# yz-cnsdqz/PSI-release

Measured on AMD Instinct MI355X. Metric: fitting iters/sec (SMPL-X+SDF+Chamfer), PROX-E batch=32, higher is better.
Workload: dtype f32

## Files before the change

psi-release_amd/csrc/fit.hip:

```cpp
#include "psi_internal.h"
#ifdef PSI_HEAD_STOPS
__device__ int psi_dbg_sstop;
#define PSI_SSTOP(k) do { if (psi_dbg_sstop == (k)) return; } while (0)
__device__ int psi_dbg_pstop;
#define PSI_PSTOP(k) do { if (psi_dbg_pstop == (k)) asm volatile("s_endpgm"); } while (0)
#define PSI_TRACE(lo, hi) PsiBlockTrace trace_((lo), (hi))
__device__ unsigned long long psi_dbg_tl[4 * 8192];
struct PsiBlockTrace {
    unsigned long long t0;
    int kind;
    int sel_lo, sel_hi;
    __device__ PsiBlockTrace(int lo = 9, int hi = 10) : t0(wall_clock64()), kind(0), sel_lo(lo), sel_hi(hi) {}
    __device__ ~PsiBlockTrace()
    {
        const unsigned bid = blockIdx.y * gridDim.x + blockIdx.x;
        if (psi_dbg_sstop < sel_lo || psi_dbg_sstop > sel_hi || threadIdx.x != 0 || bid >= 8192) return;
        unsigned long long *o = psi_dbg_tl + 4 * (size_t)bid;
        o[0] = t0;
        o[1] = wall_clock64();
        o[2] = (unsigned long long)__builtin_amdgcn_s_getreg((31 << 11) | 4) | ((unsigned long long)__builtin_amdgcn_s_getreg((31 << 11) | 20) << 32);
        o[3] = (unsigned long long)kind;
    }
};
extern "C" int psi_dbg_timeline(unsigned long long *out, int nblocks)
// ... 43 lines not shown
    const int *vid;
    const int *cs_ptr, *cs_idx;
    const int *cs_first;
    const float *scene, *sdf, *gmin, *gmax;
    const float *sdf_brick;
    const float *Wct;
    float *x, *xhr, *cam, *adam_m, *adam_v;
    int *step;
    float *h1, *h2, *o6, *betas20, *pose, *transl, *verts, *og, *gq, *fpart, *penpart, *recpart, *vppart;
    float *cverts;
    float *g_betas, *g_pose, *g_transl, *g_rot;
    unsigned long long *hx_o6, *hx_gh1;
    unsigned *hx_epoch;
    int *hx_err;
    int hc;
#ifdef PSI_HEAD_STOPS
    int stop_h, stop_t;
#define HSTOP(k) do { if (f.stop_h == (k)) return; } while (0)
#define TSTOP(k) do { if (f.stop_t == (k)) return; } while (0)
#else
#define HSTOP(k)
#define TSTOP(k)
#endif
    int *nn_hint;
    float *history;
    int max_hist;
    int fused_bwd, ncp, ncp3;
    float *glc, *gvpc, *vpc;
    float *gtc_part;
#ifndef PSI_GV_SLOTS
#define PSI_GV_SLOTS 1024
#endif
    unsigned *gvbits;
    const float *dirs_ch;
    const float *WTt_c;
    float *gA_part, *gfeat_part;
    float *spb;
    int nsv, nsv_c, nsn_m, nsn_c, spm, spc;
};

__device__ __forceinline__ float leaky(float v, float slope) { return v > 0.0f ? v : v * slope; }

__device__ __forceinline__ void gs_forward(const float *x6, float *R)
{
    float a1[3] = {x6[0], x6[2], x6[4]}, a2[3] = {x6[1], x6[3], x6[5]};
    float n1 = fmaxf(sqrtf(a1[0] * a1[0] + a1[1] * a1[1] + a1[2] * a1[2]), 1e-12f);
    float b1[3] = {a1[0] / n1, a1[1] / n1, a1[2] / n1};
    float d = b1[0] * a2[0] + b1[1] * a2[1] + b1[2] * a2[2];
    float u[3] = {a2[0] - d * b1[0], a2[1] - d * b1[1], a2[2] - d * b1[2]};
    float n2 = fmaxf(sqrtf(u[0] * u[0] + u[1] * u[1] + u[2] * u[2]), 1e-12f);
    float b2[3] = {u[0] / n2, u[1] / n2, u[2] / n2};
    float b3[3] = {b1[1] * b2[2] - b1[2] * b2[1], b1[2] * b2[0] - b1[0] * b2[2], b1[0] * b2[1] - b1[1] * b2[0]};
    for (int r = 0; r < 3; r++) {
        R[r * 3 + 0] = b1[r];
        R[r * 3 + 1] = b2[r];
        R[r * 3 + 2] = b3[r];
    }
}

__device__ __forceinline__ void gs_backward(const float *x6, const float *gR, float *g6)
{
    float a1[3] = {x6[0], x6[2], x6[4]}, a2[3] = {x6[1], x6[3], x6[5]};
    float n1 = fmaxf(sqrtf(a1[0] * a1[0] + a1[1] * a1[1] + a1[2] * a1[2]), 1e-12f);
    float b1[3] = {a1[0] / n1, a1[1] / n1, a1[2] / n1};
    float d = b1[0] * a2[0] + b1[1] * a2[1] + b1[2] * a2[2];
    float u[3] = {a2[0] - d * b1[0], a2[1] - d * b1[1], a2[2] - d * b1[2]};
// ... 327 lines not shown
#pragma unroll
            for (int a = 0; a < 3; a++) g[a] = neg[n] ? g[a] : 0.0f;
            s[n] = neg[n] ? -val : 0.0f;
        }
        if (gl) {
#pragma unroll
            for (int a = 0; a < 3; a++) gm[n][a] = g[a];
            return;
        }
        psi_st(og + (size_t)b * Vpad * 4, (unsigned)v * 16u, f4{g[0], g[1], g[2], 0.0f});
    }
    __device__ __forceinline__ void backward(int n, int b, unsigned v12, const psi_f2 (&T2)[6], const float *C)
    {
        if (!gl) return;
        const float gx = gm[n][0], gy = gm[n][1], gz = gm[n][2];
        float lx = gx, ly = gy, lz = gz;
        if (C) {
            lx = psi_dot3(C[0], C[4], C[8], gx, gy, gz);
            ly = psi_dot3(C[1], C[5], C[9], gx, gy, gz);
            lz = psi_dot3(C[2], C[6], C[10], gx, gy, gz);
        }
        psi_st(gl + (size_t)b * Npad, v12, psi_p3{lx, ly, lz});
        const float vx = psi_dot3(T2[0].x, T2[2].x, T2[4].x, lx, ly, lz), vy = psi_dot3(T2[0].y, T2[2].y, T2[4].y, lx, ly, lz),
                    vz = psi_dot3(T2[1].x, T2[3].x, T2[5].x, lx, ly, lz);
        psi_st(gvp + (size_t)b * Npad, v12, psi_p3{vx, vy, vz});
        gvmax = fmaxf(gvmax, fmaxf(fabsf(vx), fmaxf(fabsf(vy), fabsf(vz))));
        gs[n][0] = lx; gs[n][1] = ly; gs[n][2] = lz;
    }
    __device__ __forceinline__ void finish(int n, int b, int vblock, int nvb)
    {
        __shared__ psi_f2 red[PSI_SKIN_BLK / 64];
        __shared__ float red3[PSI_SKIN_BLK / 64][3];
        __shared__ float redm[PSI_SKIN_BLK / 64];
        const float ws = psi_wave_sum(s[n]);
        const float wc = (float)(int)__builtin_popcountll(__builtin_amdgcn_ballot_w64(neg[n]));
        if ((threadIdx.x & 63) == 0) red[threadIdx.x >> 6] = (psi_f2){ws, wc};
        if (gl) {
            const float sx = psi_wave_sum(gs[n][0]), sy = psi_wave_sum(gs[n][1]), sz = psi_wave_sum(gs[n][2]);
            float mx = gvmax;
#pragma unroll
            for (int o2 = 32; o2 > 0; o2 >>= 1) mx = fmaxf(mx, __shfl_xor(mx, o2, 64));
            if ((threadIdx.x & 63) == 0) {
                red3[threadIdx.x >> 6][0] = sx;
                red3[threadIdx.x >> 6][1] = sy;
                red3[threadIdx.x >> 6][2] = sz;
                redm[threadIdx.x >> 6] = mx;
            }
        }
        __syncthreads();
        if (gl && threadIdx.x == 64) {
            float mx = redm[0];
#pragma unroll
            for (int w = 1; w < PSI_SKIN_BLK / 64; w++) mx = fmaxf(mx, redm[w]);
#ifndef PSI_NO_GVMAX_ATOMIC
            if (mx > 0.0f) atomicMax(gmaxp + (blockIdx.x & (PSI_GV_SLOTS - 1)), __float_as_uint(mx));
#endif
        }
        if (threadIdx.x == 0) {
            psi_f2 a = red[0];
#pragma unroll
            for (int w = 1; w < PSI_SKIN_BLK / 64; w++) a += red[w];
            *(psi_f2 *)(penpart + ((size_t)b * nvb + vblock) * 2) = a;
        }
        if (gl && threadIdx.x < 3) {
            float a = 0.0f;
#pragma unroll
            for (int w = 0; w < PSI_SKIN_BLK / 64; w++) a += red3[w][threadIdx.x];
            gtp[((size_t)vblock * B + b) * 4 + threadIdx.x] = a;
        }
    }
};

static inline SdfPenEpilogue make_sdf_epilogue(const FitDev &f, const PsiSdfGrid &G, bool contact_vertices_only = false, const PsiLbsView *bwd = nullptr)
{
    SdfPenEpilogue e = {G, f.sdf, f.gmin, f.gmax, f.og, f.penpart, f.D, f.align_corners, f.Vpad, contact_vertices_only ? f.cs_first : nullptr,
                        {0.0f, 0.0f}, {false, false}, f.cverts, f.cs_ptr, f.cs_idx, f.n_c, nullptr, nullptr, nullptr, 0, f.B, {}, {}, 0.0f, f.gvbits};
    if (bwd) {
        e.gl = bwd->gl;
        e.gvp = bwd->g_vp;
        e.gtp = bwd->gt_part_w;
        e.Npad = bwd->m.Npad;
    }
    return e;
}

struct ContactSkinSrc {
    FitDev f;
    LbsDev m;
    const float *As, *v_posed;
    psi_f2 (*sA)[6];
    psi_f2 st[2];
    float ct;
    int v;
    float px, py, pz;
    float *sCT;
    static constexpr int NWQ = PSI_JP / 4 - 2, NWE = 10;
    f4 wq[NWE];
    int jslot;
    float (*sTR)[9] = nullptr;
    float gvm = 0.0f;
    float gs[3] = {0.0f, 0.0f, 0.0f};
// ... 94 lines not shown
            wsum3[threadIdx.x >> 6][1] = sy;
            wsum3[threadIdx.x >> 6][2] = sz;
            wmax[threadIdx.x >> 6] = mx;
        }
        __syncthreads();
        if (threadIdx.x == 64) {
            float m2 = wmax[0];
#pragma unroll
            for (int w = 1; w < psikd::QBLK / 64; w++) m2 = fmaxf(m2, wmax[w]);
#ifndef PSI_NO_GVMAX_ATOMIC
            if (m2 > 0.0f) atomicMax(f.gvbits + PSI_GV_SLOTS + (blockIdx.x & (PSI_GV_SLOTS - 1)), __float_as_uint(m2));
#endif
        }
        if (threadIdx.x < 3) {
            float a = 0.0f;
#pragma unroll
            for (int w = 0; w < psikd::QBLK / 64; w++) a += wsum3[w][threadIdx.x];
            f.gtc_part[((size_t)b * nbx + bx) * 4 + threadIdx.x] = a;
        }
    }
};

#ifdef PSI_HEAD_STOPS
extern "C" int psi_dbg_kd_mark(unsigned long long *out, int nblocks)
{
    return (int)hipMemcpyFromSymbol(out, HIP_SYMBOL(psi_kd_mark), sizeof(unsigned long long) * 4 * (size_t)(nblocks < 8192 ? nblocks : 8192));
}
extern "C" int psi_dbg_kd_reason(int *out) { return (int)hipMemcpyFromSymbol(out, HIP_SYMBOL(psi_kd_reason), sizeof(int) * 8); }
extern "C" int psi_dbg_kd_stat(int *out, int nblocks)
{
    return (int)hipMemcpyFromSymbol(out, HIP_SYMBOL(psi_kd_stat), sizeof(int) * 4 * (size_t)(nblocks < 8192 ? nblocks : 8192));
}
#endif
template <int NB>
__global__ __launch_bounds__(256, 6) void fwd_scene_kernel(FitDev f, LbsDev m, const float *__restrict__ As, const float *__restrict__ v_posed,
                                                           psikd::KdDev T, int n_kd, int nqb, int rows, float gscale, int skin_first, SdfPenEpilogue epi)
{
    extern __shared__ int smem_i[];
#ifdef PSI_HEAD_STOPS
    if (psi_dbg_sstop == 1 && (int)blockIdx.x >= n_kd) return;
    if (psi_dbg_sstop == 2 && (int)blockIdx.x < n_kd) return;
    if (psi_dbg_sstop == 3) return;
    PsiBlockTrace trace;
    if (threadIdx.x < 4 && blockIdx.x < 8192) psi_kd_stat[4 * blockIdx.x + threadIdx.x] = 0;
    trace.kind = skin_first ? ((int)blockIdx.x >= (int)gridDim.x - n_kd) : ((int)blockIdx.x < n_kd);
#endif
    int bid = blockIdx.x;
    bool is_kd;
    if (skin_first) {
        const int n_sk = (int)gridDim.x - n_kd;
        is_kd = bid >= n_sk;
        if (is_kd) bid -= n_sk;
    } else {
        is_kd = bid < n_kd;
        if (!is_kd) bid -= n_kd;
    }
    if (is_kd) {
        const int b = bid / nqb, bx = bid % nqb;
        psikd::kd_query_body<true, false>(T, ContactSkinSrc{f, m, As, v_posed, nullptr, {}, 0.0f, 0, 0.0f, 0.0f, 0.0f, nullptr, {}, 0}, f.n_c, (float *)nullptr, (int *)nullptr, f.cconst, gscale,
                                          f.fused_bwd ? (float *)nullptr : f.gq, f.fpart, f.nn_hint, rows, (const psikd::KdDev *)nullptr, (const int *)nullptr, bx, b, nqb, smem_i);
    } else {
        const int i = bid;
        psi_skin_fwd_body<NB, PsiBlendCompact>(m, As, v_posed, f.transl, f.cam, f.B, f.verts, epi, i % f.nsdfblk, (i / f.nsdfblk) * NB, f.nsdfblk);
    }
}

__global__ void contact_weight_table_kernel(const float *__restrict__ WT, int Vpad, const int *__restrict__ vid, int n_c, int J, float *__restrict__ Wct)
{
    const int i = blockIdx.x * 256 + threadIdx.x;
    if (i >= n_c * PSI_JP) return;
    const int slot = i / PSI_JP, j = i % PSI_JP;
    Wct[i] = j < J ? WT[(size_t)j * Vpad + vid[slot]] : 0.0f;
}

__global__ __launch_bounds__(1024) void loss_finalize_kernel(FitDev f, float *stats)
{
    __shared__ float red[16];
    const int t = threadIdx.x, nt = 1024;
    auto total = [&](const float *p, int n, int stride) {
        float a0 = 0, a1 = 0, a2 = 0, a3 = 0;
        int i = t;
        for (; i + 3 * nt < n; i += 4 * nt) {
            a0 += p[(size_t)i * stride];
            a1 += p[(size_t)(i + nt) * stride];
            a2 += p[(size_t)(i + 2 * nt) * stride];
            a3 += p[(size_t)(i + 3 * nt) * stride];
        }
        for (; i < n; i += nt) a0 += p[(size_t)i * stride];
        return block_sum((a0 + a1) + (a2 + a3), red);
    };
    float s_rec = total(f.recpart, f.B, 1);
    float s_vp = total(f.vppart, f.B, 1);
    float s_f = total(f.fpart, f.B * f.nfp, 1);
    float s_pen = total(f.penpart, f.B * f.nsdfblk, 2);
    float n_pen = total(f.penpart + 1, f.B * f.nsdfblk, 2);
    if (t == 0) {
// ... 563 lines not shown
    const int bz = (int)(br % nbr), by = (int)((br / nbr) % nbr), bx = (int)(br / ((size_t)nbr * nbr));
    const int ix = min(4 * bx + (l >> 4) + (c >> 2), D - 1), iy = min(4 * by + ((l >> 2) & 3) + ((c >> 1) & 1), D - 1),
              iz = min(4 * bz + (l & 3) + (c & 1), D - 1);
    dst[i] = src[((size_t)ix * D + iy) * D + iz];
}

__global__ void adam_reset_kernel(float *m, float *v, int *step, int n)
{
    int i = blockIdx.x * 256 + threadIdx.x;
    if (i < n) { m[i] = 0.0f; v[i] = 0.0f; }
    if (i == 0) *step = 0;
}

}

#ifndef PSI_GRAPH_UNROLL
#define PSI_GRAPH_UNROLL 10
#endif
constexpr int GRAPH_UNROLL = PSI_GRAPH_UNROLL;

struct psi_fit_engine {
    FitDev d;
    PsiSdfGrid grid;
    const psi_lbs_model *lbs;
    psi_nn_index *nn_index;
    float *lbs_ws;
    PsiLbsView lv;
    void *nn_ws;
    char *blob;
    float *stats_local;
    bool merged_scene;
    bool self_skin;
    bool keep_verts;
    bool scene_skin_first;
    bool fused_bwd;
    int skin_nb;
    hipGraph_t graph, graphN, graph2N;
    hipGraphExec_t graph_exec, graphN_exec, graph2N_exec;
    bool graph_ready, graphN_ready, graph2N_ready;
    hipGraph_t g_half[2];
    hipGraphExec_t ge_half[2];
    bool half_ready[2];
    const float *half_stats[2];
    hipGraph_t g_dp[2];
    hipGraphExec_t ge_dp[2];
    bool dp_ready[2];
    const void *dp_comm;
    const float *dp_stats;
    bool dp_warm;
    bool dp_no_graph;
};

static void launch_head_fwd(const FitDev &f, const PsiLbsView &lv, hipStream_t st)
{
    const dim3 g(f.B * f.hc), blk(HB);
    switch (f.hc) {
    case 8: hipLaunchKernelGGL(head_fwd_kernel<8>, g, blk, 0, st, f, lv); break;
    case 4: hipLaunchKernelGGL(head_fwd_kernel<4>, g, blk, 0, st, f, lv); break;
    case 2: hipLaunchKernelGGL(head_fwd_kernel<2>, g, blk, 0, st, f, lv); break;
    default: hipLaunchKernelGGL(head_fwd_kernel<1>, g, blk, 0, st, f, lv); break;
    }
}

template <bool ADAM>
static void launch_head_bwd(const FitDev &f, const PsiLbsView &lv, float *g_out, hipStream_t st)
{
    const dim3 g(f.B * f.hc), blk(HB);
    switch (f.hc) {
    case 8: hipLaunchKernelGGL((head_bwd_adam_kernel<8, ADAM>), g, blk, 0, st, f, lv, g_out); break;
    case 4: hipLaunchKernelGGL((head_bwd_adam_kernel<4, ADAM>), g, blk, 0, st, f, lv, g_out); break;
    case 2: hipLaunchKernelGGL((head_bwd_adam_kernel<2, ADAM>), g, blk, 0, st, f, lv, g_out); break;
    default: hipLaunchKernelGGL((head_bwd_adam_kernel<1, ADAM>), g, blk, 0, st, f, lv, g_out); break;
    }
}

static inline bool fit_use_local_stats(const FitDev &f, bool local) { return local && f.B < PSI_SKIN_MB_MIN_B; }

static int fit_forward(psi_fit_engine *e, float *stats, hipStream_t st, bool local = false, bool finalize = true)
{
    FitDev &f = e->d;
    local = e->fused_bwd ? (local || !finalize) : fit_use_local_stats(f, local);
    launch_head_fwd(f, e->lv, st);
    PSI_CHECK_LAUNCH("head_fwd_kernel");
    psi_mark("head_fwd_kernel", st);
    int rc = psi_lbs_blend_forward(e->lbs, f.B, e->lbs_ws, st);
    if (rc) return rc;
    float gscale = f.w_contact / ((f.indep ? 1.0f : (float)f.B * (float)f.world) * (float)f.n_c);
    if (e->nn_index && e->merged_scene) {
        const psikd::KdDev T = psi_nn_index_dev(e->nn_index);
        const int nqb = f.nfp, n_kd = nqb * f.B;
        FitDev fk = f;
        if (!e->keep_verts) fk.verts = nullptr;
        if (e->skin_nb == 2)
            hipLaunchKernelGGL(fwd_scene_kernel<2>, dim3(n_kd + f.nsdfblk * psi_cdiv(f.B, 2)), dim3(256), psikd::kd_lds_bytes(T.rows), st, fk, e->lv.m,
                               e->lv.A, e->lv.v_posed, T, n_kd, nqb, T.rows, gscale, e->scene_skin_first ? 1 : 0, make_sdf_epilogue(f, e->grid, false, e->fused_bwd ? &e->lv : nullptr));
        else
            hipLaunchKernelGGL(fwd_scene_kernel<1>, dim3(n_kd + f.nsdfblk * f.B), dim3(256), psikd::kd_lds_bytes(T.rows), st, fk, e->lv.m, e->lv.A,
                               e->lv.v_posed, T, n_kd, nqb, T.rows, gscale, e->scene_skin_first ? 1 : 0, make_sdf_epilogue(f, e->grid, false, e->fused_bwd ? &e->lv : nullptr));
        PSI_CHECK_LAUNCH("fwd_scene_kernel");
        psi_mark("fwd_scene_kernel", st);
        if (local) return 0;
        hipLaunchKernelGGL(loss_finalize_kernel, dim3(1), dim3(1024), 0, st, f, stats);
        PSI_CHECK_LAUNCH("loss_finalize_kernel");
        psi_mark("loss_finalize_kernel", st);
        return 0;
    }
    const bool all_verts = !e->nn_index || (getenv("PSI_KEEP_VERTS") && getenv("PSI_KEEP_VERTS")[0] == '1');
    if (e->skin_nb == 2)
        hipLaunchKernelGGL((psi_skin_fwd_kernel<SdfPenEpilogue, 2>), dim3(f.nsdfblk, psi_cdiv(f.B, 2)), dim3(PSI_SKIN_BLK), 0, st, e->lv.m, e->lv.A,
                           e->lv.v_posed, f.transl, f.cam, f.B, f.verts, make_sdf_epilogue(f, e->grid, !all_verts));
    else
        hipLaunchKernelGGL((psi_skin_fwd_kernel<SdfPenEpilogue, 1>), dim3(f.nsdfblk, f.B), dim3(PSI_SKIN_BLK), 0, st, e->lv.m, e->lv.A,
                           e->lv.v_posed, f.transl, f.cam, f.B, f.verts, make_sdf_epilogue(f, e->grid, !all_verts));
    PSI_CHECK_LAUNCH("skin_fwd_sdf_kernel");
    psi_mark("skin_fwd_sdf_kernel", st);
    if (e->nn_index && !all_verts)
        rc = psi_nn_index_contact(e->nn_index, f.cverts, (long)f.n_c * 3, nullptr, f.B, f.n_c, f.cconst, gscale, f.gq, f.fpart, f.nn_hint, st);
    else if (e->nn_index)
        rc = psi_nn_index_contact(e->nn_index, f.verts, (long)f.V * 3, f.vid, f.B, f.n_c, f.cconst, gscale, f.gq, f.fpart, f.nn_hint, st);
    else
        rc = psi_nn_contact(f.verts, (long)f.V * 3, f.vid, f.scene, f.B, f.n_c, f.m, e->nn_ws, f.cconst, gscale, f.gq, f.fpart, nullptr, st);
    if (rc) return rc;
    if (local) return 0;
    hipLaunchKernelGGL(loss_finalize_kernel, dim3(1), dim3(1024), 0, st, f, stats);
    PSI_CHECK_LAUNCH("loss_finalize_kernel");
    psi_mark("loss_finalize_kernel", st);
    return 0;
}

static int fit_launch_stats(psi_fit_engine *e, float *stats, hipStream_t st)
{
// ... 139 lines not shown
    memcpy(b3p.data(), h_b3, NJ6 * 4);
    for (int o = 0; o < NH; o++) for (int k = 0; k < NZ; k++) W1T[(size_t)k * NH + o] = h_w1[(size_t)o * NZ + k];
    for (int o = 0; o < NH; o++) for (int k = 0; k < NH; k++) W2T[(size_t)k * NH + o] = h_w2[(size_t)o * NH + k];
    for (int o = 0; o < NJ6; o++) for (int k = 0; k < NH; k++) W3T[(size_t)k * 128 + o] = h_w3[(size_t)o * NH + k];
    std::vector<int> cs_ptr(V + 1, 0), cs_idx(f.n_c), cs_first(V, 0);
    for (int i = 0; i < f.n_c; i++) cs_ptr[h_contact_ids[i] + 1]++;
    for (int v = 0; v < V; v++) cs_ptr[v + 1] += cs_ptr[v];
    {
        std::vector<int> fill(cs_ptr.begin(), cs_ptr.end() - 1);
        for (int i = 0; i < f.n_c; i++) cs_idx[fill[h_contact_ids[i]]++] = i;
        for (int v = 0; v < V; v++)
            if (cs_ptr[v + 1] > cs_ptr[v]) cs_first[v] = cs_idx[cs_ptr[v]] | (std::min(cs_ptr[v + 1] - cs_ptr[v], 127) << 24);
    }
    struct Item { const void *src; size_t bytes; size_t off; };
    std::vector<Item> items;
    size_t o = 0;
    auto take = [&](size_t bytes) { size_t r = o; o += (bytes + 255) & ~(size_t)255; return r; };
    auto cst = [&](const void *src, size_t bytes) { size_t r = take(bytes); items.push_back({src, bytes, r}); return r; };
    size_t o_w1t = cst(W1T.data(), W1T.size() * 4), o_b1 = cst(h_b1, NH * 4), o_w2t = cst(W2T.data(), W2T.size() * 4), o_b2 = cst(h_b2, NH * 4),
           o_w3t = cst(W3T.data(), W3T.size() * 4), o_b3 = cst(b3p.data(), 128 * 4), o_w1 = cst(h_w1, (size_t)NH * NZ * 4),
           o_w2 = cst(h_w2, (size_t)NH * NH * 4), o_w3 = cst(h_w3, (size_t)NJ6 * NH * 4), o_lh = cst(h_lh_comp, (size_t)f.ncomp * 45 * 4),
           o_rh = cst(h_rh_comp, (size_t)f.ncomp * 45 * 4), o_pm = cst(h_pose_mean, (size_t)J * 3 * 4), o_vid = cst(h_contact_ids, (size_t)f.n_c * 4),
           o_cp = cst(cs_ptr.data(), cs_ptr.size() * 4), o_ci = cst(cs_idx.data(), cs_idx.size() * 4), o_cf = cst(cs_first.data(), cs_first.size() * 4), o_gmin = cst(h_gmin, 12), o_gmax = cst(h_gmax, 12);
    size_t zero_begin = o;
    size_t o_x = take((size_t)B * XD * 4), o_xhr = take((size_t)B * XD * 4), o_cam = take((size_t)B * 16 * 4), o_am = take((size_t)B * XD * 4),
           o_av = take((size_t)B * XD * 4), o_step = take(256), o_h1 = take((size_t)B * NH * 4), o_h2 = take((size_t)B * NH * 4),
           o_o6 = take((size_t)B * 128 * 4), o_b20 = take((size_t)B * NB * 4), o_pose = take((size_t)B * J * 3 * 4), o_tr = take((size_t)B * 3 * 4),
           o_verts = take((size_t)B * V * 3 * 4), o_cv = take((size_t)B * f.n_c * 3 * 4), o_og = take((size_t)B * psi_cdiv(V, 256) * 256 * 4 * 4),
           o_gq = take((size_t)B * f.n_c * 3 * 4), o_fp = take((size_t)B * f.nfp * 4), o_pp = take((size_t)B * f.nsdfblk * 2 * 4),
           o_rp = take((size_t)B * 4), o_vp = take((size_t)B * 4), o_gb = take((size_t)B * NB * 4), o_gp = take((size_t)B * J * 3 * 4),
           o_gt = take((size_t)B * 3 * 4), o_gr = take((size_t)B * J * 9 * 4), o_hist = take((size_t)f.max_hist * 4 * 4), o_stats = take(256), o_hint = take((size_t)B * f.n_c * 4);
    size_t o_hxo = take((size_t)B * f.hc * 128 * 8), o_hxg = take((size_t)B * f.hc * NH * 8), o_hxc = take((size_t)2 * B * 4);
    size_t o_wct = take((size_t)f.n_c * PSI_JP * 4);
    e->fused_bwd = e->merged_scene && !(getenv("PSI_FIT_FUSED_BWD") && getenv("PSI_FIT_FUSED_BWD")[0] == '0');
    f.fused_bwd = e->fused_bwd ? 1 : 0;
    f.ncp = psi_cdiv(f.n_c, 256) * 256;
    f.ncp3 = 3 * f.ncp;
    size_t o_glc = 0, o_gvpc = 0, o_vpc = 0, o_gtc = 0, o_gvb = 0, o_wttc = 0, o_dirsc = 0, o_gap = 0, o_gfp = 0, o_spb = 0;
    {
        PsiLbsView lv0;
        if (int rcv = psi_lbs_view(lbs, B, reinterpret_cast<float *>((uintptr_t)4096), &lv0)) { delete e; return rcv; }
        const int Kpad = lv0.m.Kpad, Npad = lv0.m.Npad, nsn = lv0.nsn;
        const int SM = Npad / 16, SC = f.ncp3 / 16;
        f.nsv = lv0.nsv;
        f.nsv_c = f.ncp / 256;
        f.nsn_c = 0;
        for (int c = 1, best = INT_MAX; c < nsn; c++) {
            const int longest = std::max(psi_cdiv(SM, nsn - c), psi_cdiv(SC, c));
            if (longest < best) { best = longest; f.nsn_c = c; }
        }
        f.nsn_m = nsn - f.nsn_c;
        f.spm = psi_cdiv(SM, f.nsn_m);
        f.spc = f.nsn_c ? psi_cdiv(SC, f.nsn_c) : 0;
        if (e->fused_bwd && !f.nsn_c) { e->fused_bwd = false; f.fused_bwd = 0; }
        if (e->fused_bwd) {
            o_glc = take((size_t)B * f.ncp3 * 4); o_gvpc = take((size_t)B * f.ncp3 * 4); o_vpc = take((size_t)B * f.ncp3 * 4);
            o_gtc = take((size_t)B * f.nfp * 4 * 4); o_gvb = take(2 * PSI_GV_SLOTS * 4); o_wttc = take((size_t)f.ncp * PSI_JP * 4); o_dirsc = take((size_t)f.ncp3 * Kpad * 4);
            o_gap = take((size_t)(f.nsv + f.nsv_c) * B * PSI_JP * 16 * 4); o_gfp = take((size_t)(f.nsn_m + f.nsn_c) * B * Kpad * 4);
            o_spb = take((size_t)B * 4);
        }
    }
    const bool bricks = (cfg->D % 4 == 0) && cfg->D <= (PSI_SDF_CELLS ? 480 : 800) && !(getenv("PSI_SDF_LINEAR") && getenv("PSI_SDF_LINEAR")[0] == '1');
#if PSI_SDF_CELLS
    size_t o_brick = bricks ? take((size_t)f.D * f.D * f.D * 32) : 0;
#else
    size_t o_brick = bricks ? take((size_t)(f.D / 4) * (f.D / 4) * (f.D / 4) * PSI_BRICK_FLOATS * 4) : 0;
// ... 6 lines not shown
        psi_set_error("psi_fit_create: hipMalloc(%zu) failed: %s", o, hipGetErrorString(err));
        return (int)err;
    }
    err = hipMemset(e->blob + zero_begin, 0, o - zero_begin);
    if (err == hipSuccess) err = hipMemset(e->blob + o_hint, 0xff, (size_t)B * f.n_c * 4);
    for (auto &it : items)
        if (err == hipSuccess) err = hipMemcpy(e->blob + it.off, it.src, it.bytes, hipMemcpyHostToDevice);
    if (err != hipSuccess) {
        (void)hipFree(e->blob);
        delete e;
        psi_set_error("psi_fit_create: upload failed: %s", hipGetErrorString(err));
        return (int)err;
    }
    char *bl = e->blob;
    auto F = [&](size_t off) { return (float *)(bl + off); };
    f.W1T = F(o_w1t); f.b1 = F(o_b1); f.W2T = F(o_w2t); f.b2 = F(o_b2); f.W3T = F(o_w3t); f.b3 = F(o_b3);
    f.W1 = F(o_w1); f.W2 = F(o_w2); f.W3 = F(o_w3); f.lhc = F(o_lh); f.rhc = F(o_rh); f.pose_mean = F(o_pm);
    f.vid = (const int *)(bl + o_vid); f.cs_ptr = (const int *)(bl + o_cp); f.cs_idx = (const int *)(bl + o_ci); f.cs_first = (const int *)(bl + o_cf);
    f.gmin = F(o_gmin); f.gmax = F(o_gmax);
    f.x = F(o_x); f.xhr = F(o_xhr); f.cam = F(o_cam); f.adam_m = F(o_am); f.adam_v = F(o_av); f.step = (int *)(bl + o_step); f.hx_err = f.step + 1;
    f.h1 = F(o_h1); f.h2 = F(o_h2); f.o6 = F(o_o6); f.betas20 = F(o_b20); f.pose = F(o_pose); f.transl = F(o_tr);
    f.verts = F(o_verts); f.cverts = F(o_cv); f.og = F(o_og); f.gq = F(o_gq); f.fpart = F(o_fp); f.penpart = F(o_pp);
    f.recpart = F(o_rp); f.vppart = F(o_vp); f.g_betas = F(o_gb); f.g_pose = F(o_gp); f.g_transl = F(o_gt); f.g_rot = F(o_gr);
    f.history = F(o_hist);
    f.nn_hint = (int *)(bl + o_hint);
    f.hx_o6 = (unsigned long long *)(bl + o_hxo); f.hx_gh1 = (unsigned long long *)(bl + o_hxg); f.hx_epoch = (unsigned *)(bl + o_hxc);
    e->stats_local = F(o_stats);
    e->lbs_ws = F(o_lws);
    {
        int rcv = psi_lbs_view(lbs, B, e->lbs_ws, &e->lv);
        if (rcv) { (void)hipFree(e->blob); delete e; return rcv; }
    }
    f.Wct = F(o_wct);
    if (e->fused_bwd) {
        f.glc = F(o_glc); f.gvpc = F(o_gvpc); f.vpc = F(o_vpc); f.gtc_part = F(o_gtc); f.WTt_c = F(o_wttc); f.dirs_ch = F(o_dirsc); f.gvbits = (unsigned *)(bl + o_gvb);
        f.gA_part = F(o_gap); f.gfeat_part = F(o_gfp); f.spb = F(o_spb);
    }
    e->scene_skin_first = getenv("PSI_SCENE_ORDER") && getenv("PSI_SCENE_ORDER")[0] == '1';
    e->skin_nb = cfg->B > 128 && !e->lv.m.Wc ? 2 : 1;
    if (const char *nbv = getenv("PSI_SKIN_NB")) e->skin_nb = atoi(nbv) == 2 ? 2 : 1;
    hipLaunchKernelGGL(contact_weight_table_kernel, dim3(psi_cdiv((long)f.n_c * PSI_JP, 256)), dim3(256), 0, 0, e->lv.m.WT, e->lv.m.Vpad, f.vid,
                       f.n_c, J, (float *)f.Wct);
    if (e->fused_bwd) {
        hipLaunchKernelGGL(contact_weight_tiles_kernel, dim3(psi_cdiv((long)f.ncp * PSI_JP, 256)), dim3(256), 0, 0, f.Wct, f.n_c, f.ncp, (float *)f.WTt_c);
        hipLaunchKernelGGL(contact_dirs_h_kernel, dim3(psi_cdiv((long)f.ncp3 * e->lv.m.Kpad, 256)), dim3(256), 0, 0, e->lv.m.dirs_bh, e->lv.m.Kpad, f.vid,
                           f.n_c, f.ncp3, (float *)f.dirs_ch);
    }
    f.sdf_brick = nullptr;
    if (bricks) {
#if PSI_SDF_CELLS
        const size_t n = (size_t)f.D * f.D * f.D * 8;
        hipLaunchKernelGGL(sdf_to_cells_kernel, dim3((unsigned)psi_cdiv((long)n, 256)), dim3(256), 0, 0, d_sdf, F(o_brick), f.D);
#else
        const size_t n = (size_t)(f.D / 4) * (f.D / 4) * (f.D / 4) * PSI_BRICK_FLOATS;
        hipLaunchKernelGGL(sdf_to_bricks_kernel, dim3((unsigned)psi_cdiv((long)n, 256)), dim3(256), 0, 0, d_sdf, F(o_brick), f.D);
#endif
        f.sdf_brick = F(o_brick);
    }
    e->grid = psi_sdf_grid_make(f.sdf_brick, h_gmin, h_gmax, f.D, f.align_corners);
    err = hipDeviceSynchronize();
    if (err == hipSuccess) err = hipGetLastError();
    if (err != hipSuccess) {
        (void)hipFree(e->blob);
        delete e;
        psi_set_error("psi_fit_create: layout kernels failed: %s", hipGetErrorString(err));
        return (int)err;
    }
    e->nn_ws = bl + o_nws;
    if (cfg->nn_mode == 1) {
        std::vector<float> hs((size_t)f.m * 3);
        err = hipMemcpy(hs.data(), d_scene_verts, hs.size() * 4, hipMemcpyDeviceToHost);
        int rc = err == hipSuccess ? psi_nn_index_create(&e->nn_index, hs.data(), f.m) : (int)err;
        if (rc) {
            (void)hipFree(e->blob);
            delete e;
            return rc;
        }
    }
    *out = e;
    return 0;
}

extern "C" void psi_fit_destroy(psi_fit_engine *e)
{
    if (!e) return;
    if (e->nn_index) psi_nn_index_destroy(e->nn_index);
    if (e->graph_ready) {
        (void)hipGraphExecDestroy(e->graph_exec);
        (void)hipGraphDestroy(e->graph);
    }
    if (e->graphN_ready) {
        (void)hipGraphExecDestroy(e->graphN_exec);
        (void)hipGraphDestroy(e->graphN);
    }
    if (e->graph2N_ready) {
        (void)hipGraphExecDestroy(e->graph2N_exec);
        (void)hipGraphDestroy(e->graph2N);
    }
    for (int i = 0; i < 2; i++) {
        if (e->half_ready[i]) {
            (void)hipGraphExecDestroy(e->ge_half[i]);
            (void)hipGraphDestroy(e->g_half[i]);
        }
        if (e->dp_ready[i]) {
            (void)hipGraphExecDestroy(e->ge_dp[i]);
            (void)hipGraphDestroy(e->g_dp[i]);
        }
    }
    (void)hipFree(e->blob);
    delete e;
}
// ... 357 lines not shown
```

psi-release_amd/csrc/lbs_device.h:

```cpp
#pragma once
#ifndef PSI_TRACE
#define PSI_TRACE(lo, hi)
#endif
#ifndef PSI_SSTOP
#define PSI_SSTOP(k)
#endif
#ifndef PSI_PSTOP
#define PSI_PSTOP(k)
#endif
#include <hip/hip_runtime.h>

typedef float psi_f4 __attribute__((ext_vector_type(4)));

constexpr int PSI_JP = 64;
constexpr int PSI_SUB_MAX = PSI_JP * (PSI_JP + 1) / 2;
constexpr int PSI_ITEM_MAX = 2 * PSI_JP;
constexpr int PSI_NJUMP = 6;
constexpr int PSI_WNZ = 8;
constexpr int PSI_A_TAIL = 16;

struct LbsDev {
    int V, J, NB, P, K, Kpad, N, Npad, Vpad, maxlevel, njump;
    int dirs_tile;
    float dirs_unscale;
// ... 424 lines not shown
    r += __shfl_xor(r, 1, 64);
    r += __shfl_xor(r, 2, 64);
    return r;
}
template <int MAXS>
__device__ __forceinline__ float psi_sum_slices_split(const float *__restrict__ p, size_t stride, int n, int s0)
{
    float v[MAXS];
    psi_slices_load<MAXS>(p, stride, n, s0, v);
    return psi_slices_sum<MAXS>(v, p, stride, n, s0);
}


typedef float psi_f2 __attribute__((ext_vector_type(2)));
constexpr int PSI_SKIN_BLK = 256;

template <int CTRL, int ROWS>
__device__ __forceinline__ float psi_dpp(float x)
{
    return __builtin_bit_cast(float, __builtin_amdgcn_update_dpp(0, __builtin_bit_cast(int, x), CTRL, ROWS, 0xf, false));
}
__device__ __forceinline__ float psi_wave_sum(float x)
{
    x += psi_dpp<0xB1, 0xf>(x);
    x += psi_dpp<0x4E, 0xf>(x);
    x += psi_dpp<0x124, 0xf>(x);
    x += psi_dpp<0x128, 0xf>(x);
    x += psi_dpp<0x142, 0xa>(x);
    x += psi_dpp<0x143, 0xc>(x);
    return __builtin_bit_cast(float, __builtin_amdgcn_readlane(__builtin_bit_cast(int, x), 63));
}

struct psi_p3 { float x, y, z; };
template <class T>
__device__ __forceinline__ T psi_ld(const void *uniform_base, unsigned lane_off)
{
    return *(const T *)((const char *)uniform_base + lane_off);
}
template <class T>
__device__ __forceinline__ void psi_st(void *uniform_base, unsigned lane_off, const T &val)
{
    *(T *)((char *)uniform_base + lane_off) = val;
}

#ifndef PSI_DENSE_UNROLL
#define PSI_DENSE_UNROLL 11
#endif
enum PsiBlendForm { PsiBlendCompact = 0, PsiBlendPipelined = 1 };
template <int NB>
__device__ __forceinline__ psi_f2 (*psi_transform_stage())[PSI_JP][6]
{
    __shared__ psi_f2 sA[NB][PSI_JP][6];
    return sA;
}
template <int NB>
struct PsiBlendN {
    psi_f2 st[NB][2];
    float wk[PSI_WNZ];
    unsigned jk[PSI_WNZ / 4];
    const float *As_b[NB];
    typedef psi_f2 (*Staged)[PSI_JP][6];
    __device__ __forceinline__ void issue(const LbsDev &m, const float *__restrict__ As, const int (&b)[NB], int v)
    {
#pragma unroll
        for (int n = 0; n < NB; n++) As_b[n] = As + (size_t)b[n] * m.J * 12;
        if (m.Wc) {
#pragma unroll
            for (int n = 0; n < NB; n++)
#pragma unroll
                for (int q = 0; q < 2; q++) {
                    const int idx = threadIdx.x + q * PSI_SKIN_BLK;
                    st[n][q] = idx < m.J * 6 ? *(const psi_f2 *)(As_b[n] + idx * 2) : (psi_f2){0.0f, 0.0f};
                }
            const __amdgpu_buffer_rsrc_t rc = __builtin_amdgcn_make_buffer_rsrc((void *)m.Wc, 0, PSI_WNZ * m.Vpad * 4, 0x00020000);
            const __amdgpu_buffer_rsrc_t rj = __builtin_amdgcn_make_buffer_rsrc((void *)m.Wj, 0, PSI_WNZ / 4 * m.Vpad * 4, 0x00020000);
#pragma unroll
            for (int k = 0; k < PSI_WNZ; k++)
                wk[k] = __builtin_bit_cast(float, __builtin_amdgcn_raw_buffer_load_b32(rc, (unsigned)v * 4u, (unsigned)(k * m.Vpad) * 4u, 0));
#pragma unroll
            for (int k = 0; k < PSI_WNZ / 4; k++) jk[k] = __builtin_amdgcn_raw_buffer_load_b32(rj, (unsigned)v * 4u, (unsigned)(k * m.Vpad) * 4u, 0);
        }
    }
    __device__ __forceinline__ Staged commit(const LbsDev &m)
    {
        const Staged sA = psi_transform_stage<NB>();
        if (!m.Wc) return sA;
#pragma unroll
        for (int n = 0; n < NB; n++)
#pragma unroll
            for (int q = 0; q < 2; q++) {
                const int idx = threadIdx.x + q * PSI_SKIN_BLK;
                if (idx < m.J * 6) (&sA[n][0][0])[idx] = st[n][q];
            }
        __syncthreads();
        return sA;
    }
    template <PsiBlendForm FORM = PsiBlendCompact>
    __device__ __forceinline__ void blend(const LbsDev &m, Staged sA, int v, psi_f2 (&T2)[NB][6]) const
    {
#pragma unroll
        for (int n = 0; n < NB; n++)
#pragma unroll
            for (int e = 0; e < 6; e++) T2[n][e] = (psi_f2){0.0f, 0.0f};
        if (m.Wc) {
#pragma unroll
            for (int k = 0; k < PSI_WNZ; k++) {
                if (__builtin_amdgcn_ballot_w64(wk[k] != 0.0f) == 0) break;
                psi_f2 w2 = {wk[k], wk[k]};
                const int jj = (jk[k >> 2] >> (8 * (k & 3))) & 0xff;
#pragma unroll
                for (int n = 0; n < NB; n++)
#pragma unroll
                    for (int e = 0; e < 6; e++) T2[n][e] = __builtin_elementwise_fma(w2, sA[n][jj][e], T2[n][e]);
            }
            return;
        }
        const psi_f2 *Ab[NB];
#pragma unroll
        for (int n = 0; n < NB; n++) Ab[n] = (const psi_f2 *)As_b[n];
        const __amdgpu_buffer_rsrc_t rw = __builtin_amdgcn_make_buffer_rsrc((void *)m.WTt, 0, PSI_JP * m.Vpad * 4, 0x00020000);
        const unsigned v4 = (unsigned)(v & 63) * 4u;
        const unsigned tile_off = (unsigned)__builtin_amdgcn_readfirstlane(v >> 6) * (unsigned)(PSI_JP * 64 * 4);
        auto wload = [&](int k, unsigned ro) { return __builtin_bit_cast(float, __builtin_amdgcn_raw_buffer_load_b32(rw, v4 + k * 256, ro, 0)); };
        unsigned ro = tile_off;
// ... 75 lines not shown
            } else {
#pragma nounroll
                for (int g = 0; g < ngroups; g++) group(g);
            }
        }
    }
};
typedef PsiBlendN<1> PsiBlend;

__device__ __forceinline__ float psi_dot3p(float a, float b, float c, float d, float x, float y, float z)
{
    return __builtin_fmaf(c, z, __builtin_fmaf(b, y, a * x)) + d;
}
__device__ __forceinline__ float psi_dot3(float a, float b, float c, float x, float y, float z)
{
    return __builtin_fmaf(c, z, __builtin_fmaf(b, y, a * x));
}

struct PsiSkinNoEpilogue {
    __device__ __forceinline__ void backward(int, int, unsigned, const psi_f2 (&)[6], const float *) {}
    __device__ __forceinline__ void store(float *verts, size_t body_off, int, int, unsigned v12, float x, float y, float z) const
    {
        if (verts) psi_st(verts + body_off, v12, psi_p3{x, y, z});
    }
    __device__ __forceinline__ void vertex(int, int, int, float, float, float, bool) {}
    __device__ __forceinline__ void finish(int, int, int, int) {}
};

template <int NB, PsiBlendForm FORM, class Epi>
__device__ __forceinline__ void psi_skin_fwd_body(const LbsDev &m, const float *__restrict__ As, const float *__restrict__ v_posed,
                                                  const float *__restrict__ transl, const float *__restrict__ cam_ext, int B,
                                                  float *__restrict__ verts, Epi &epi, int vblock, int b0, int nvb)
{
    const int v = vblock * PSI_SKIN_BLK + threadIdx.x;
    const bool live = v < m.V;
    const unsigned v12 = (unsigned)v * 12u;
    int bs[NB];
#pragma unroll
    for (int n = 0; n < NB; n++) bs[n] = min(b0 + n, B - 1);
    PsiBlendN<NB> bl;
    bl.issue(m, As, bs, v);
    psi_p3 pp[NB];
#pragma unroll
    for (int n = 0; n < NB; n++) pp[n] = psi_ld<psi_p3>(v_posed + (size_t)bs[n] * m.Npad, v12);
    psi_f2 T2[NB][6];
    bl.template blend<FORM>(m, bl.commit(m), v, T2);
#pragma unroll
    for (int n = 0; n < NB; n++) {
        const int b = bs[n];
        const bool on = n == 0 || b0 + n < B;
        const float px = pp[n].x, py = pp[n].y, pz = pp[n].z;
        float x = psi_dot3p(T2[n][0].x, T2[n][0].y, T2[n][1].x, T2[n][1].y, px, py, pz);
        float y = psi_dot3p(T2[n][2].x, T2[n][2].y, T2[n][3].x, T2[n][3].y, px, py, pz);
        float z = psi_dot3p(T2[n][4].x, T2[n][4].y, T2[n][5].x, T2[n][5].y, px, py, pz);
        if (transl) {
            x += transl[(size_t)b * 3 + 0];
            y += transl[(size_t)b * 3 + 1];
            z += transl[(size_t)b * 3 + 2];
        }
        if (cam_ext) {
            const float *C = cam_ext + (size_t)b * 16;
            float X = psi_dot3p(C[0], C[1], C[2], C[3], x, y, z);
            float Y = psi_dot3p(C[4], C[5], C[6], C[7], x, y, z);
            float Z = psi_dot3p(C[8], C[9], C[10], C[11], x, y, z);
            x = X; y = Y; z = Z;
        }
        epi.vertex(n, b, v, x, y, z, live && on);
// ... 234 lines not shown
```

Before: 10420.

## Replace static skin-block grid with persistent sharded work pool in scene kernel

The fused scene kernel used to launch one block per kd-search query block plus one per skin/SDF tile. Now it launches only the kd blocks plus an occupancy-sized set of extra blocks. Every block, the kd blocks included once they finish searching, pulls skin tiles from sharded atomic counters that reset themselves, and the first tile of each extra block is placed statically. The aim is to cut block-launch and tail-imbalance cost and let search blocks help with skinning. It adds atomic contention, a per-tile syncthreads, and asm tricks that keep the thread index and kernel args opaque to the compiler. The gvmax slot index is changed to use a tile id instead of blockIdx.

```diff
diff --git a/psi-release_amd/csrc/fit.hip b/psi-release_amd/csrc/fit.hip
--- a/psi-release_amd/csrc/fit.hip
+++ b/psi-release_amd/csrc/fit.hip
@@ -99,6 +99,7 @@
 #define PSI_GV_SLOTS 1024
 #endif
     unsigned *gvbits;
+    unsigned *pool;
     const float *dirs_ch;
     const float *WTt_c;
     float *gA_part, *gfeat_part;
@@ -492,41 +493,42 @@
         __shared__ psi_f2 red[PSI_SKIN_BLK / 64];
         __shared__ float red3[PSI_SKIN_BLK / 64][3];
         __shared__ float redm[PSI_SKIN_BLK / 64];
+        const unsigned tid = psi_tid();
         const float ws = psi_wave_sum(s[n]);
         const float wc = (float)(int)__builtin_popcountll(__builtin_amdgcn_ballot_w64(neg[n]));
-        if ((threadIdx.x & 63) == 0) red[threadIdx.x >> 6] = (psi_f2){ws, wc};
+        if ((tid & 63) == 0) red[tid >> 6] = (psi_f2){ws, wc};
         if (gl) {
             const float sx = psi_wave_sum(gs[n][0]), sy = psi_wave_sum(gs[n][1]), sz = psi_wave_sum(gs[n][2]);
             float mx = gvmax;
 #pragma unroll
             for (int o2 = 32; o2 > 0; o2 >>= 1) mx = fmaxf(mx, __shfl_xor(mx, o2, 64));
-            if ((threadIdx.x & 63) == 0) {
-                red3[threadIdx.x >> 6][0] = sx;
-                red3[threadIdx.x >> 6][1] = sy;
-                red3[threadIdx.x >> 6][2] = sz;
-                redm[threadIdx.x >> 6] = mx;
+            if ((tid & 63) == 0) {
+                red3[tid >> 6][0] = sx;
+                red3[tid >> 6][1] = sy;
+                red3[tid >> 6][2] = sz;
+                redm[tid >> 6] = mx;
             }
         }
         __syncthreads();
-        if (gl && threadIdx.x == 64) {
+        if (gl && tid == 64) {
             float mx = redm[0];
 #pragma unroll
             for (int w = 1; w < PSI_SKIN_BLK / 64; w++) mx = fmaxf(mx, redm[w]);
 #ifndef PSI_NO_GVMAX_ATOMIC
-            if (mx > 0.0f) atomicMax(gmaxp + (blockIdx.x & (PSI_GV_SLOTS - 1)), __float_as_uint(mx));
+            if (mx > 0.0f) atomicMax(gmaxp + ((b * nvb + vblock) & (PSI_GV_SLOTS - 1)), __float_as_uint(mx));
 #endif
         }
-        if (threadIdx.x == 0) {
+        if (tid == 0) {
             psi_f2 a = red[0];
 #pragma unroll
             for (int w = 1; w < PSI_SKIN_BLK / 64; w++) a += red[w];
             *(psi_f2 *)(penpart + ((size_t)b * nvb + vblock) * 2) = a;
         }
-        if (gl && threadIdx.x < 3) {
+        if (gl && tid < 3) {
             float a = 0.0f;
 #pragma unroll
-            for (int w = 0; w < PSI_SKIN_BLK / 64; w++) a += red3[w][threadIdx.x];
-            gtp[((size_t)vblock * B + b) * 4 + threadIdx.x] = a;
+            for (int w = 0; w < PSI_SKIN_BLK / 64; w++) a += red3[w][tid];
+            gtp[((size_t)vblock * B + b) * 4 + tid] = a;
         }
     }
 };
@@ -687,36 +689,82 @@
     return (int)hipMemcpyFromSymbol(out, HIP_SYMBOL(psi_kd_stat), sizeof(int) * 4 * (size_t)(nblocks < 8192 ? nblocks : 8192));
 }
 #endif
+#ifndef PSI_POOL_SHARDS
+#define PSI_POOL_SHARDS 8
+#endif
+#ifdef PSI_HEAD_STOPS
+__device__ unsigned long long psi_dbg_tile[2 * 8192];
+extern "C" int psi_dbg_tiles(unsigned long long *out, int ntiles)
+{
+    return (int)hipMemcpyFromSymbol(out, HIP_SYMBOL(psi_dbg_tile), sizeof(unsigned long long) * 2 * (size_t)(ntiles < 8192 ? ntiles : 8192));
+}
+#endif
+template <class K>
+__device__ __forceinline__ const K &psi_kernarg_trip(const K &arg)
+{
+    int z = 0;
+    asm volatile("" : "+s"(z));
+    return (&arg)[z];
+}
 template <int NB>
 __global__ __launch_bounds__(256, 6) void fwd_scene_kernel(FitDev f, LbsDev m, const float *__restrict__ As, const float *__restrict__ v_posed,
-                                                           psikd::KdDev T, int n_kd, int nqb, int rows, float gscale, int skin_first, SdfPenEpilogue epi)
+                                                           psikd::KdDev T, int n_kd, int nqb, int rows, float gscale, SdfPenEpilogue epi)
 {
     extern __shared__ int smem_i[];
+    const int bid = blockIdx.x;
+    bool search = bid < n_kd;
 #ifdef PSI_HEAD_STOPS
-    if (psi_dbg_sstop == 1 && (int)blockIdx.x >= n_kd) return;
-    if (psi_dbg_sstop == 2 && (int)blockIdx.x < n_kd) return;
+    if (psi_dbg_sstop == 1 && !search) return;
+    if (psi_dbg_sstop == 2) search = false;
     if (psi_dbg_sstop == 3) return;
     PsiBlockTrace trace;
     if (threadIdx.x < 4 && blockIdx.x < 8192) psi_kd_stat[4 * blockIdx.x + threadIdx.x] = 0;
-    trace.kind = skin_first ? ((int)blockIdx.x >= (int)gridDim.x - n_kd) : ((int)blockIdx.x < n_kd);
+    trace.kind = bid < n_kd;
 #endif
-    int bid = blockIdx.x;
-    bool is_kd;
-    if (skin_first) {
-        const int n_sk = (int)gridDim.x - n_kd;
-        is_kd = bid >= n_sk;
-        if (is_kd) bid -= n_sk;
-    } else {
-        is_kd = bid < n_kd;
-        if (!is_kd) bid -= n_kd;
-    }
-    if (is_kd) {
+    if (search) {
         const int b = bid / nqb, bx = bid % nqb;
         psikd::kd_query_body<true, false>(T, ContactSkinSrc{f, m, As, v_posed, nullptr, {}, 0.0f, 0, 0.0f, 0.0f, 0.0f, nullptr, {}, 0}, f.n_c, (float *)nullptr, (int *)nullptr, f.cconst, gscale,
                                           f.fused_bwd ? (float *)nullptr : f.gq, f.fpart, f.nn_hint, rows, (const psikd::KdDev *)nullptr, (const int *)nullptr, bx, b, nqb, smem_i);
-    } else {
-        const int i = bid;
-        psi_skin_fwd_body<NB, PsiBlendCompact>(m, As, v_posed, f.transl, f.cam, f.B, f.verts, epi, i % f.nsdfblk, (i / f.nsdfblk) * NB, f.nsdfblk);
+#ifdef PSI_HEAD_STOPS
+        if (psi_dbg_sstop == 1) return;
+#endif
+    }
+    const int n_tiles = f.nsdfblk * ((f.B + NB - 1) / NB);
+    const int d0 = min((int)gridDim.x - n_kd, n_tiles);
+    const int ns = min((int)gridDim.x, PSI_POOL_SHARDS), s = bid % ns;
+    const int lo = d0 + (int)((long)(n_tiles - d0) * s / ns), hi = d0 + (int)((long)(n_tiles - d0) * (s + 1) / ns);
+    const unsigned members = (gridDim.x - (unsigned)s + (unsigned)ns - 1) / (unsigned)ns;
+    const bool placed = bid >= n_kd && bid - n_kd < d0;
+    unsigned *head = f.pool + 64 * s, *done = head + 32;
+    __shared__ int s_tile[2];
+    for (int k = 0; k <= hi - lo + 1; k++) {
+        int t;
+        if (placed && k == 0) {
+            t = bid - n_kd;
+        } else {
+            if (threadIdx.x == 0) {
+                const int c = lo + (int)atomicAdd(head, 1u);
+                s_tile[k & 1] = c < hi ? c : -1;
+                if (c >= hi && atomicAdd(done, 1u) == members - 1) {
+                    atomicExch(head, 0u);
+                    atomicExch(done, 0u);
+                }
+            }
+            __syncthreads();
+            t = __builtin_amdgcn_readfirstlane(s_tile[k & 1]);
+            if (t < 0) break;
+        }
+#ifdef PSI_HEAD_STOPS
+        if (threadIdx.x == 0 && t < 8192 && psi_dbg_sstop >= 9) psi_dbg_tile[2 * t] = wall_clock64();
+#endif
+        const FitDev &ft = psi_kernarg_trip(f);
+        SdfPenEpilogue e = psi_kernarg_trip(epi);
+        psi_skin_fwd_body<NB, PsiBlendCompact>(psi_kernarg_trip(m), As, v_posed, ft.transl, ft.cam, ft.B, ft.verts, e, t % ft.nsdfblk, (t / ft.nsdfblk) * NB,
+                                               ft.nsdfblk);
+#ifdef PSI_HEAD_STOPS
+        if (threadIdx.x == 0 && t < 8192 && psi_dbg_sstop >= 9) psi_dbg_tile[2 * t + 1] = wall_clock64();
+        trace.kind += 256;
+#endif
     }
 }
 
@@ -1346,7 +1394,8 @@
     bool merged_scene;
     bool self_skin;
     bool keep_verts;
-    bool scene_skin_first;
+    int scene_pool;
+    int scene_pool_knob;
     bool fused_bwd;
     int skin_nb;
     hipGraph_t graph, graphN, graph2N;
@@ -1390,6 +1439,19 @@
 
 static inline bool fit_use_local_stats(const FitDev &f, bool local) { return local && f.B < PSI_SKIN_MB_MIN_B; }
 
+static void size_scene_pool(psi_fit_engine *e)
+{
+    const FitDev &f = e->d;
+    const size_t lds = psikd::kd_lds_bytes(psi_nn_index_dev(e->nn_index).rows);
+    const long n_kd = (long)f.nfp * f.B, n_tiles = (long)f.nsdfblk * psi_cdiv(f.B, e->skin_nb);
+    int dev = 0, ncu = 0, per_cu = 0;
+    (void)hipGetDevice(&dev);
+    (void)hipDeviceGetAttribute(&ncu, hipDeviceAttributeMultiprocessorCount, dev);
+    if (e->skin_nb == 2) (void)hipOccupancyMaxActiveBlocksPerMultiprocessor(&per_cu, fwd_scene_kernel<2>, 256, lds);
+    else (void)hipOccupancyMaxActiveBlocksPerMultiprocessor(&per_cu, fwd_scene_kernel<1>, 256, lds);
+    e->scene_pool = (int)std::min(std::max((long)per_cu * ncu - n_kd, 1L), n_tiles);
+}
+
 static int fit_forward(psi_fit_engine *e, float *stats, hipStream_t st, bool local = false, bool finalize = true)
 {
     FitDev &f = e->d;
@@ -1405,12 +1467,15 @@
         const int nqb = f.nfp, n_kd = nqb * f.B;
         FitDev fk = f;
         if (!e->keep_verts) fk.verts = nullptr;
+        const size_t lds = psikd::kd_lds_bytes(T.rows);
+        const int n_tiles = f.nsdfblk * psi_cdiv(f.B, e->skin_nb);
+        const int S = std::min(e->scene_pool_knob >= 0 ? e->scene_pool_knob : e->scene_pool, n_tiles);
         if (e->skin_nb == 2)
-            hipLaunchKernelGGL(fwd_scene_kernel<2>, dim3(n_kd + f.nsdfblk * psi_cdiv(f.B, 2)), dim3(256), psikd::kd_lds_bytes(T.rows), st, fk, e->lv.m,
-                               e->lv.A, e->lv.v_posed, T, n_kd, nqb, T.rows, gscale, e->scene_skin_first ? 1 : 0, make_sdf_epilogue(f, e->grid, false, e->fused_bwd ? &e->lv : nullptr));
+            hipLaunchKernelGGL(fwd_scene_kernel<2>, dim3(n_kd + S), dim3(256), lds, st, fk, e->lv.m, e->lv.A, e->lv.v_posed, T, n_kd, nqb, T.rows,
+                               gscale, make_sdf_epilogue(f, e->grid, false, e->fused_bwd ? &e->lv : nullptr));
         else
-            hipLaunchKernelGGL(fwd_scene_kernel<1>, dim3(n_kd + f.nsdfblk * f.B), dim3(256), psikd::kd_lds_bytes(T.rows), st, fk, e->lv.m, e->lv.A,
-                               e->lv.v_posed, T, n_kd, nqb, T.rows, gscale, e->scene_skin_first ? 1 : 0, make_sdf_epilogue(f, e->grid, false, e->fused_bwd ? &e->lv : nullptr));
+            hipLaunchKernelGGL(fwd_scene_kernel<1>, dim3(n_kd + S), dim3(256), lds, st, fk, e->lv.m, e->lv.A, e->lv.v_posed, T, n_kd, nqb, T.rows,
+                               gscale, make_sdf_epilogue(f, e->grid, false, e->fused_bwd ? &e->lv : nullptr));
         PSI_CHECK_LAUNCH("fwd_scene_kernel");
         psi_mark("fwd_scene_kernel", st);
         if (local) return 0;
@@ -1616,6 +1681,7 @@
            o_gt = take((size_t)B * 3 * 4), o_gr = take((size_t)B * J * 9 * 4), o_hist = take((size_t)f.max_hist * 4 * 4), o_stats = take(256), o_hint = take((size_t)B * f.n_c * 4);
     size_t o_hxo = take((size_t)B * f.hc * 128 * 8), o_hxg = take((size_t)B * f.hc * NH * 8), o_hxc = take((size_t)2 * B * 4);
     size_t o_wct = take((size_t)f.n_c * PSI_JP * 4);
+    size_t o_pool = take(PSI_POOL_SHARDS * 2 * 128);
     e->fused_bwd = e->merged_scene && !(getenv("PSI_FIT_FUSED_BWD") && getenv("PSI_FIT_FUSED_BWD")[0] == '0');
     f.fused_bwd = e->fused_bwd ? 1 : 0;
     f.ncp = psi_cdiv(f.n_c, 256) * 256;
@@ -1688,11 +1754,13 @@
         if (rcv) { (void)hipFree(e->blob); delete e; return rcv; }
     }
     f.Wct = F(o_wct);
+    f.pool = (unsigned *)(bl + o_pool);
     if (e->fused_bwd) {
         f.glc = F(o_glc); f.gvpc = F(o_gvpc); f.vpc = F(o_vpc); f.gtc_part = F(o_gtc); f.WTt_c = F(o_wttc); f.dirs_ch = F(o_dirsc); f.gvbits = (unsigned *)(bl + o_gvb);
         f.gA_part = F(o_gap); f.gfeat_part = F(o_gfp); f.spb = F(o_spb);
     }
-    e->scene_skin_first = getenv("PSI_SCENE_ORDER") && getenv("PSI_SCENE_ORDER")[0] == '1';
+    e->scene_pool = 1;
+    e->scene_pool_knob = getenv("PSI_SCENE_POOL") ? std::max(atoi(getenv("PSI_SCENE_POOL")), 0) : -1;
     e->skin_nb = cfg->B > 128 && !e->lv.m.Wc ? 2 : 1;
     if (const char *nbv = getenv("PSI_SKIN_NB")) e->skin_nb = atoi(nbv) == 2 ? 2 : 1;
     hipLaunchKernelGGL(contact_weight_table_kernel, dim3(psi_cdiv((long)f.n_c * PSI_JP, 256)), dim3(256), 0, 0, e->lv.m.WT, e->lv.m.Vpad, f.vid,
@@ -1733,6 +1801,7 @@
             return rc;
         }
     }
+    if (e->nn_index && e->merged_scene) size_scene_pool(e);
     *out = e;
     return 0;
 }
diff --git a/psi-release_amd/csrc/lbs_device.h b/psi-release_amd/csrc/lbs_device.h
--- a/psi-release_amd/csrc/lbs_device.h
+++ b/psi-release_amd/csrc/lbs_device.h
@@ -480,6 +480,12 @@
 }
 
 struct psi_p3 { float x, y, z; };
+__device__ __forceinline__ unsigned psi_tid()
+{
+    unsigned t = threadIdx.x;
+    asm volatile("" : "+v"(t));
+    return t;
+}
 template <class T>
 __device__ __forceinline__ T psi_ld(const void *uniform_base, unsigned lane_off)
 {
@@ -517,7 +523,7 @@
             for (int n = 0; n < NB; n++)
 #pragma unroll
                 for (int q = 0; q < 2; q++) {
-                    const int idx = threadIdx.x + q * PSI_SKIN_BLK;
+                    const int idx = psi_tid() + q * PSI_SKIN_BLK;
                     st[n][q] = idx < m.J * 6 ? *(const psi_f2 *)(As_b[n] + idx * 2) : (psi_f2){0.0f, 0.0f};
                 }
             const __amdgpu_buffer_rsrc_t rc = __builtin_amdgcn_make_buffer_rsrc((void *)m.Wc, 0, PSI_WNZ * m.Vpad * 4, 0x00020000);
@@ -537,7 +543,7 @@
         for (int n = 0; n < NB; n++)
 #pragma unroll
             for (int q = 0; q < 2; q++) {
-                const int idx = threadIdx.x + q * PSI_SKIN_BLK;
+                const int idx = psi_tid() + q * PSI_SKIN_BLK;
                 if (idx < m.J * 6) (&sA[n][0][0])[idx] = st[n][q];
             }
         __syncthreads();
@@ -679,7 +685,7 @@
                                                   const float *__restrict__ transl, const float *__restrict__ cam_ext, int B,
                                                   float *__restrict__ verts, Epi &epi, int vblock, int b0, int nvb)
 {
-    const int v = vblock * PSI_SKIN_BLK + threadIdx.x;
+    const int v = vblock * PSI_SKIN_BLK + psi_tid();
     const bool live = v < m.V;
     const unsigned v12 = (unsigned)v * 12u;
     int bs[NB];
```

New measurement: 10890, median of 6. +4.5%, better.
